# shanpenghui/ExtractORB

Hardware: AMD Instinct MI355X
Metric: frames/sec (ORB extract, 640x480x8-level x1000 feat) (higher is better)
Workload: dtype u8; 1 GPU; mono640: 640x480 mono stream, 8 levels, 1000 features, synthetic noise frames; variant=noise, nfeatures=1000, nlevels=8, handles_per_gpu=1, parallelism=frames sharded 512/GPU

## Files before the change

### extractorb_amd/csrc/k_describe_body.hpp

```cpp
#pragma once
#include <hip/hip_runtime.h>
#include <stdint.h>

#include "orbx_device.hpp"
#include "k_blur_body.hpp"

namespace orbx {
constexpr int kUmaxStatic[16] = {15, 15, 15, 15, 14, 14, 14, 13, 13, 12, 11, 10, 9, 8, 6, 3};
static __constant__ int c_umax[16] = {15, 15, 15, 15, 14, 14, 14, 13, 13, 12, 11, 10, 9, 8, 6, 3};
static __constant__ __attribute__((aligned(16))) float c_patternF[1024] = {
#include "orbx_brief_pattern.inc"
};

__device__ __forceinline__ float fastAtan2Deg(float y, float x) {
    const float sc = (float)(180.0 / 3.1415926535897932384626433832795);
    const float p1 = 0.9997878412794807f * sc, p3 = -0.3258083974640975f * sc, p5 = 0.1555786518463281f * sc,
                p7 = -0.04432655554792128f * sc;
    const float eps = (float)2.2204460492503131e-16;
    const float ax = fabsf(x), ay = fabsf(y);
    float a, c, c2;
    if (ax >= ay) {
        c = __fdiv_rn(ay, __fadd_rn(ax, eps));
        c2 = __fmul_rn(c, c);
        a = __fmul_rn(__fadd_rn(__fmul_rn(__fadd_rn(__fmul_rn(__fadd_rn(__fmul_rn(p7, c2), p5), c2), p3), c2), p1), c);
    } else {
        c = __fdiv_rn(ax, __fadd_rn(ay, eps));
        c2 = __fmul_rn(c, c);
        a = __fsub_rn(90.f, __fmul_rn(__fadd_rn(__fmul_rn(__fadd_rn(__fmul_rn(__fadd_rn(__fmul_rn(p7, c2), p5), c2), p3), c2), p1), c));
    }
    if (x < 0) a = __fsub_rn(180.f, a);
    if (y < 0) a = __fsub_rn(360.f, a);
    return a;
}

__device__ __forceinline__ void sincosGlibc(float y, float* s_out, float* c_out) {
    const double hpi_inv = 0x1.45F306DC9C883p+23, hpi = 0x1.921FB54442D18p0;
    const double C0 = 0x1p0, C1 = -0x1.ffffffd0c621cp-2, C2 = 0x1.55553e1068f19p-5, C3 = -0x1.6c087e89a359dp-10,
                 C4 = 0x1.99343027bf8c3p-16;
    const double S1 = -0x1.555545995a603p-3, S2 = 0x1.1107605230bc4p-7, S3 = -0x1.994eb3774cf24p-13;
    double x = (double)y;
    const unsigned top12 = (__float_as_uint(y) >> 20) & 0x7ff;
    int n = 0;
    if (top12 < 0x3f4) {
        if (top12 < 0x398) { *s_out = y; *c_out = 1.0f; return; }
    } else {
        const double r = __dmul_rn(x, hpi_inv);
        n = ((int)r + 0x800000) >> 24;
        x = __dsub_rn(x, __dmul_rn((double)n, hpi));
    }
    const double x2 = __dmul_rn(x, x);
    auto polySin = [&](double xx) {
        const double x3 = __dmul_rn(xx, x2), s1 = __dadd_rn(S2, __dmul_rn(x2, S3)), x7 = __dmul_rn(x3, x2),
                     s = __dadd_rn(xx, __dmul_rn(x3, S1));
        return __dadd_rn(s, __dmul_rn(x7, s1));
    };
    auto polyCos = [&](double sg) {
        const double x4 = __dmul_rn(x2, x2), c2 = __dadd_rn(sg * C3, __dmul_rn(x2, sg * C4)),
                     c1 = __dadd_rn(sg * C0, __dmul_rn(x2, sg * C1)), x6 = __dmul_rn(x4, x2),
                     c = __dadd_rn(c1, __dmul_rn(x4, sg * C2));
        return __dadd_rn(c, __dmul_rn(x6, c2));
    };
    const bool odd = (n & 1) != 0;
    const int ns = odd ? n + 1 : n, nc = odd ? n : n + 1;
    const double sgnS = ((ns & 3) == 1 || (ns & 3) == 2) ? -1.0 : 1.0;
    const float ps = (float)polySin(x * sgnS), pc = (float)polyCos((nc & 2) ? -1.0 : 1.0);
    *s_out = odd ? pc : ps;
    *c_out = odd ? ps : pc;
}

constexpr int kDescWaves = 4;
constexpr int kBriefReach = 18;
constexpr int kRawRows = 2 * kHalfPatch + 1;
constexpr int kRawStride = 40;
constexpr int kBlurRows = 2 * kBriefReach + 1;
constexpr int kBlurStride = 40;
constexpr int kPatchLds = kRawRows * kRawStride + kBlurRows * kBlurStride;
constexpr int kPbRows = 2 * (kBriefReach + 3) + 1;
constexpr int kPbStride = 44;
constexpr int kPbRawBytes = (kPbRows * kPbStride + 15) & ~15;
constexpr int kPbLds = kPbRawBytes + kBlurRows * kBlurStride;
static __constant__ unsigned c_pbRun[32] = {
    0x0b0700, 0x0c1200, 0x080301, 0x0b0b01, 0x0c1601, 0x0c0102, 0x0c0d02, 0x0b1902, 0x050003, 0x0c0503, 0x091103, 0x0b1a03, 0x050004, 0x0c0504, 0x081104,
    0x0c1904, 0x060005, 0x0c0605, 0x091205, 0x0a1b05, 0x050006, 0x0c0506, 0x0c1106, 0x081d06, 0x0b0207, 0x0b0d07, 0x0b1807, 0x0c0508, 0x0c1108, 0x031d08, 0x010c09, 0x0c0d09};

#if defined(ORBX_DESC_STAMPS) && defined(ORBX_DESCRIBE_TU)
__device__ unsigned long long g_descStamps[6 * 1024];
extern "C" int orbx_debug_desc_stamps(unsigned long long* out) { return (int)hipMemcpyFromSymbol(out, HIP_SYMBOL(g_descStamps), sizeof(g_descStamps)); }
#define DSTAMP(i) do { const int dsW = (int)blockIdx.y * 4 + (int)(threadIdx.x >> 6); \
        if ((threadIdx.x & 63) == 0 && blockIdx.x == 0 && blockIdx.z == 0 && dsW < 1024) g_descStamps[6 * dsW + (i)] = __builtin_amdgcn_s_memrealtime(); } while (0)
#else
#define DSTAMP(i) do {} while (0)
#endif
template <bool PB>
struct DescLds {
    static constexpr int kPatches = 2 * kDescWaves * (PB ? kPbLds : kPatchLds), kWtabWords = 2 * 16 * (PB ? 12 : 8);
    static constexpr int kWtabOff = (kPatches + 15) & ~15, kBytes = kWtabOff + 4 * kWtabWords;
};

template <bool PB>
__device__ __forceinline__ void describeBlock(const LevelGeom* __restrict__ lv, int nlevels,
                                              const uint8_t* __restrict__ pyr, const uint8_t* __restrict__ blur,
                                              const uint2* __restrict__ sel, int selPerFrame,
                                              const int* __restrict__ levelCount, const int* __restrict__ levelLap,
                                              Keypoint* __restrict__ outK, uint8_t* __restrict__ outD, int capacity,
                                              int* __restrict__ nOut, int* __restrict__ monoOut,
                                              Keypoint* __restrict__ outLevelK, int* __restrict__ outLevelCounts, int fewWaves,
                                              uint8_t* smem, unsigned (*wtab)[16][PB ? 12 : 8], int chunk, int f, int levelLo, int levelHi) {
    const int tid = threadIdx.x, wave = tid >> 6, lane = tid & 63, half = lane >> 5, hl = lane & 31;
    DSTAMP(0);
    if constexpr (PB) {
        for (int e = tid; e < 2 * 16 * 12; e += 256) {
            const int which = e / 192, a = (e / 12) & 15, j = e % 12;
            unsigned w = 0;
#pragma unroll
            for (int b = 0; b < 4; b++) {
                const int u = 4 * j + b - (kBriefReach + 4), au = u < 0 ? -u : u;
                if (au <= kHalfPatch && au <= c_umax[a]) w |= (unsigned)(which ? 1 : u + 16) << (8 * b);
            }
            wtab[which][a][j] = w;
        }
    } else {
        const int which = tid >> 7, a = (tid >> 3) & 15, j = tid & 7;
        unsigned w = 0;
#pragma unroll
        for (int b = 0; b < 4; b++) {
            const int u = 4 * j + b - kHalfPatch, au = u < 0 ? -u : u;
            if (au <= c_umax[a]) w |= (unsigned)(which ? 1 : u + 16) << (8 * b);
        }
        wtab[which][a][j] = w;
    }
    __syncthreads();
    const int slot0 = __builtin_amdgcn_readfirstlane((chunk * kDescWaves + wave) * 2);
    const int slot = slot0 + half;
    int total = 0, totalLap = 0, level = 0, seqBase = 0, lapBase = 0, levelN, selOff;
    if (fewWaves) {
        int myOff = 0x7fffffff, myCnt = 0, myLap = 0;
        if (lane < nlevels) { myOff = lv[lane].selOff; myCnt = levelCount[f * nlevels + lane]; myLap = levelLap[f * nlevels + lane]; }
        int incC = myCnt, incL = myLap;
        static_assert(kMaxLevels == 16, "the scan below covers one DPP row of 16 lanes");
        incC += __builtin_amdgcn_update_dpp(0, incC, 0x111, 0xF, 0xF, true); incL += __builtin_amdgcn_update_dpp(0, incL, 0x111, 0xF, 0xF, true);
        incC += __builtin_amdgcn_update_dpp(0, incC, 0x112, 0xF, 0xF, true); incL += __builtin_amdgcn_update_dpp(0, incL, 0x112, 0xF, 0xF, true);
        incC += __builtin_amdgcn_update_dpp(0, incC, 0x114, 0xF, 0xF, true); incL += __builtin_amdgcn_update_dpp(0, incL, 0x114, 0xF, 0xF, true);
        incC += __builtin_amdgcn_update_dpp(0, incC, 0x118, 0xF, 0xF, true); incL += __builtin_amdgcn_update_dpp(0, incL, 0x118, 0xF, 0xF, true);
        total = __builtin_amdgcn_readlane(incC, kMaxLevels - 1); totalLap = __builtin_amdgcn_readlane(incL, kMaxLevels - 1);
        level = __popcll(__ballot(slot0 >= myOff)) - 1;
        seqBase = __builtin_amdgcn_readlane(incC - myCnt, level); lapBase = __builtin_amdgcn_readlane(incL - myLap, level);
        levelN = __builtin_amdgcn_readlane(myCnt, level); selOff = __builtin_amdgcn_readlane(myOff, level);
        if (slot0 == 0 && outLevelCounts && lane < nlevels) outLevelCounts[f * nlevels + lane] = myCnt;
    } else {
        for (int l = 0; l < nlevels; l++) {
            const int c = levelCount[f * nlevels + l], lp = levelLap[f * nlevels + l];
            if (slot0 >= lv[l].selOff) { level = l; seqBase = total; lapBase = totalLap; }
            total += c;
            totalLap += lp;
        }
        selOff = lv[level].selOff;
        levelN = levelCount[f * nlevels + level];
        if (slot0 == 0 && outLevelCounts && lane < nlevels) outLevelCounts[f * nlevels + lane] = levelCount[f * nlevels + lane];
    }
    if (slot0 == 0 && lane == 0) { nOut[f] = total; monoOut[f] = total - totalLap; }
    if (level < levelLo || level >= levelHi) return;
    const int i = slot - selOff;
    const bool active = slot < selPerFrame && i < levelN;
    if (__ballot(active) == 0) return;
    DSTAMP(1);
    const int gw = lv[level].w, gh = lv[level].h, pyrStride = lv[level].pyrStride, blurStride = lv[level].blurStride;
    const uint8_t* pyrL = pyr + lv[level].pyrOff + (long long)f * lv[level].pyrFrameBytes;
    const uint8_t* blurL = blur + lv[level].blurOff + (long long)f * lv[level].blurFrameBytes;
    const uint2 e = active ? sel[(long long)f * selPerFrame + slot] : make_uint2(0u, 0u);
    int kx = e.x & 0xffff, ky = e.x >> 16;
    const float response = (float)(e.y >> 24);
    kx = min(max(kx, kEdge), gw - kEdge - 1);
    ky = min(max(ky, kEdge), gh - kEdge - 1);

    DSTAMP(2);
    int m10 = 0, m01 = 0;
    uint8_t* blurT;
    int blurMis;
    unsigned pbRun = 0;
    if constexpr (PB) pbRun = c_pbRun[hl];
    if constexpr (PB) {
        uint8_t* rawT = smem + (wave * 2 + half) * kPbLds;
        blurT = rawT + kPbRawBytes;
        blurMis = 0;
        constexpr int kSteps = (kPbRows + 3) / 4;
        const int l8 = hl & 7, rsub = hl >> 3;
        const int col0 = kPadL + kx - (kBriefReach + 4), mis = col0 & 3;
        const int rOff = __mul24(kEdge + ky - (kBriefReach + 3) + rsub, pyrStride) + (col0 - mis) + 8 * l8;
        uint2 wr[kSteps];
#pragma unroll
        for (int s = 0; s < kSteps; s++) {
            wr[s] = uint2{0u, 0u};
            if (l8 < 6 && rsub + 4 * s < kPbRows) __builtin_memcpy(&wr[s], pyrL + ((unsigned)rOff + (unsigned)(4 * s * pyrStride)), 8);
        }
        uint8_t* rdst = rawT + rsub * kPbStride + 8 * l8;
#pragma unroll
        for (int s = 0; s < kSteps; s++) {
            const unsigned nxt = (unsigned)__builtin_amdgcn_update_dpp(0, (int)wr[s].x, 0x101, 0xF, 0xF, false);
            const unsigned v0 = __builtin_amdgcn_alignbyte(wr[s].y, wr[s].x, (unsigned)mis), v1 = __builtin_amdgcn_alignbyte(nxt, wr[s].y, (unsigned)mis);
            if (l8 < 6 && rsub + 4 * s < kPbRows) {
                *(unsigned*)(rdst + 4 * s * kPbStride) = v0;
                if (l8 < 5) *(unsigned*)(rdst + 4 * s * kPbStride + 4) = v1;
            }
        }
        asm volatile("" ::: "memory");
        __builtin_amdgcn_fence(__ATOMIC_ACQ_REL, "wavefront");
        __builtin_amdgcn_wave_barrier();
        asm volatile("" ::: "memory");
        DSTAMP(3);
        if (hl < kRawRows) {
            const int v = hl - kHalfPatch, a = v < 0 ? -v : v;
            const unsigned* row = (const unsigned*)(rawT + (hl + 6) * kPbStride);
            unsigned s1 = 0, s0 = 0;
#pragma unroll
            for (int j = 1; j <= 9; j++) {
                const unsigned px = row[j];
                s1 = __builtin_amdgcn_udot4(px, wtab[0][a][j], s1, false);
                s0 = __builtin_amdgcn_udot4(px, wtab[1][a][j], s0, false);
            }
            m10 = (int)s1 - 16 * (int)s0;
            m01 = v * (int)s0;
        }
        {
            const int g4 = (int)(pbRun & 0xff), o0 = (int)((pbRun >> 8) & 0xff), nOut = (int)(pbRun >> 16);
            const uint8_t* src = rawT + o0 * kPbStride + 4 * g4;
            uint8_t* dst = blurT + o0 * kBlurStride + 4 * g4;
            blurRun(nOut,
                    [&](int i, unsigned& d0, unsigned& d1, unsigned& d2) {
                        const unsigned* row = (const unsigned*)(src + min(i, nOut + 5) * kPbStride);
                        d0 = row[0]; d1 = row[1]; d2 = row[2];
                    },
                    [&](int rr, unsigned word) { *(unsigned*)(dst + rr * kBlurStride) = word; });
        }
        asm volatile("" ::: "memory");
        __builtin_amdgcn_fence(__ATOMIC_ACQ_REL, "wavefront");
        __builtin_amdgcn_wave_barrier();
        asm volatile("" ::: "memory");
    } else {
    uint8_t* rawT = smem + (wave * 2 + half) * kPatchLds;
    blurT = rawT + kRawRows * kRawStride;
    const int rawCol0 = kPadL + kx - kHalfPatch, rawMis = rawCol0 & 3;
    const int blurCol0 = kx - kBriefReach;
    blurMis = blurCol0 & 3;
    {
        constexpr int kPairs = 5, kRowsPerStep = 6;
        static_assert(kRawStride == 8 * kPairs && kBlurStride == 8 * kPairs, "tile rows are five 8-byte pairs");
        constexpr int kRawSteps = (kRawRows + kRowsPerStep - 1) / kRowsPerStep, kBlurSteps = (kBlurRows + kRowsPerStep - 1) / kRowsPerStep;
        const int rr = (hl * 52) >> 8, rc = hl - rr * kPairs;
        const bool stLane = hl < kRowsPerStep * kPairs;
        const int rOff = __mul24(kEdge + ky - kHalfPatch + rr, pyrStride) + (rawCol0 - rawMis) + 8 * rc;
        const int bOff = __mul24(ky - kBriefReach + rr, blurStride) + (blurCol0 - blurMis) + 8 * rc;
        uint2 wr[kRawSteps], wb[kBlurSteps];
#pragma unroll
        for (int s = 0; s < kRawSteps; s++) {
            wr[s] = uint2{0u, 0u};
            if (stLane && rr + kRowsPerStep * s < kRawRows) __builtin_memcpy(&wr[s], pyrL + ((unsigned)rOff + (unsigned)(kRowsPerStep * s * pyrStride)), 8);
        }
#pragma unroll
        for (int s = 0; s < kBlurSteps; s++) {
            wb[s] = uint2{0u, 0u};
            if (stLane && rr + kRowsPerStep * s < kBlurRows) __builtin_memcpy(&wb[s], blurL + ((unsigned)bOff + (unsigned)(kRowsPerStep * s * blurStride)), 8);
        }
        uint8_t* rdst = rawT + rr * kRawStride + 8 * rc;
        uint8_t* bdst = blurT + rr * kBlurStride + 8 * rc;
#pragma unroll
        for (int s = 0; s < kRawSteps; s++)
            if (stLane && rr + kRowsPerStep * s < kRawRows) *(uint2*)(rdst + kRowsPerStep * s * kRawStride) = wr[s];
#pragma unroll
        for (int s = 0; s < kBlurSteps; s++)
            if (stLane && rr + kRowsPerStep * s < kBlurRows) *(uint2*)(bdst + kRowsPerStep * s * kBlurStride) = wb[s];
    }
    asm volatile("" ::: "memory");
    __builtin_amdgcn_fence(__ATOMIC_ACQ_REL, "wavefront");
    __builtin_amdgcn_wave_barrier();
    asm volatile("" ::: "memory");

    DSTAMP(3);
    if (hl < kRawRows) {
        const int v = hl - kHalfPatch, a = v < 0 ? -v : v;
        const unsigned* row = (const unsigned*)(rawT + hl * kRawStride);
        unsigned d[9];
#pragma unroll
        for (int j = 0; j < 9; j++) d[j] = row[j];
        unsigned s1 = 0, s0 = 0;
#pragma unroll
        for (int j = 0; j < 8; j++) {
            const unsigned px = __builtin_amdgcn_alignbyte(d[j + 1], d[j], (unsigned)rawMis);
            s1 = __builtin_amdgcn_udot4(px, wtab[0][a][j], s1, false);
            s0 = __builtin_amdgcn_udot4(px, wtab[1][a][j], s0, false);
        }
        m10 = (int)s1 - 16 * (int)s0;
        m01 = v * (int)s0;
    }
    }
    auto rowSum = [](int v) {
        v += __builtin_amdgcn_update_dpp(0, v, 0xB1, 0xF, 0xF, false);
        v += __builtin_amdgcn_update_dpp(0, v, 0x4E, 0xF, 0xF, false);
        v += __builtin_amdgcn_update_dpp(0, v, 0x141, 0xF, 0xF, false);
        v += __builtin_amdgcn_update_dpp(0, v, 0x140, 0xF, 0xF, false);
        return v;
    };
    m10 = rowSum(m10); m01 = rowSum(m01);
    m10 += __shfl_xor(m10, 16);
    m01 += __shfl_xor(m01, 16);
    const float angle = fastAtan2Deg((float)m01, (float)m10);

    const float factorPI = (float)(3.1415926535897932384626433832795 / 180.0);
    float a, b;
    sincosGlibc(__fmul_rn(angle, factorPI), &b, &a);
    const uint8_t* bc = blurT + kBriefReach * kBlurStride + blurMis + kBriefReach;
    unsigned myWord = 0;
#pragma unroll
    for (int j = 0; j < 8; j++) {
        const int p = hl + 32 * j;
        const float4 pt = ((const float4*)c_patternF)[p];
        const float x0 = pt.x, y0 = pt.y, x1 = pt.z, y1 = pt.w;
        const int r0 = (int)rintf(__fadd_rn(__fmul_rn(x0, b), __fmul_rn(y0, a)));
        const int q0 = (int)rintf(__fsub_rn(__fmul_rn(x0, a), __fmul_rn(y0, b)));
        const int r1 = (int)rintf(__fadd_rn(__fmul_rn(x1, b), __fmul_rn(y1, a)));
        const int q1 = (int)rintf(__fsub_rn(__fmul_rn(x1, a), __fmul_rn(y1, b)));
        const int t0 = bc[__mul24(r0, kBlurStride) + q0], t1 = bc[__mul24(r1, kBlurStride) + q1];
        const unsigned long long m = __ballot(t0 < t1);
        const unsigned mine = half ? (unsigned)(m >> 32) : (unsigned)m;
        myWord = hl == j ? mine : myWord;
    }
    DSTAMP(4);
    if (!active) return;

    const int lapRank = (int)(e.y & 0x7fffff), isLap = (int)((e.y >> 23) & 1);
    const int lapBefore = lapBase + lapRank;
    const int monoBefore = (seqBase - lapBase) + (i - lapRank);
    const int at = isLap ? total - 1 - lapBefore : monoBefore;
    float ox = (float)kx, oy = (float)ky;
    const float scale = lv[level].scale;
    if (level != 0) { ox = __fmul_rn(ox, scale); oy = __fmul_rn(oy, scale); }
    const float patchSize = (float)lv[level].patchSize;
    if (at < capacity) {
        if (hl == 0) {
            Keypoint k;
            k.x = ox; k.y = oy; k.size = patchSize; k.angle = angle; k.response = response;
            k.octave = level; k.class_id = -1;
            outK[(long long)f * capacity + at] = k;
        }
        if (hl < 8) ((unsigned*)(outD + ((long long)f * capacity + at) * 32))[hl] = myWord;
    }
    if (outLevelK && hl == 0 && seqBase + i < capacity) {
        Keypoint k;
        k.x = (float)kx; k.y = (float)ky; k.size = patchSize; k.angle = angle; k.response = response;
        k.octave = level; k.class_id = -1;
        outLevelK[(long long)f * capacity + seqBase + i] = k;
    }
}


}
```

### extractorb_amd/csrc/orbx_api.cpp

```cpp
#include "orbx_internal.hpp"

static_assert(sizeof(orbx_keypoint) == sizeof(Keypoint), "orbx_keypoint layout");
static_assert(sizeof(orbx_proj_query) == sizeof(ProjQuery), "orbx_proj_query layout");

double g_hostT[8];
long g_hostN;
const bool g_hostTiming = getenv("ORBX_HOST_TIMING") && atoi(getenv("ORBX_HOST_TIMING")) != 0;
TestAids g_aids;
const char* const kSlotNames[ORBX_NUM_KERNELS] = {"k_pyr_first", "k_resize", "k_blur", "k_fast",
                                            "k_octree", "k_describe", "memset+copies", "batch_total",
                                            "k_stereo_rows+match+filter", "k_frame_finish+k_search_init+k_search_proj"};
thread_local std::string g_createError;

namespace {
constexpr int kSplitRatioNum = 3, kSplitRatioDen = 2;

void freeAll(orbx_handle* h) {
    void* dev[] = {h->d_input, h->d_pyr, h->d_blur, h->d_candPos, h->d_candSeg, h->d_cellCount, h->d_cellOff, h->d_nodeOf, h->d_candCount, h->d_sink, h->d_sel, h->d_levelCount,
                   h->d_levelLap, h->d_lap, h->d_lv, h->d_cells, h->d_rx, h->d_ry, h->d_xq, h->d_cols, h->d_colLevels, h->d_colCoef, h->d_foot, h->d_tiles, h->d_laneItem, h->d_out,
                   h->d_octArena, h->d_leafHist, h->d_leafBest, h->d_leafCode, h->d_bowWord, h->d_bowNode, h->d_bowWeight, h->d_rowOff, h->d_sadDist,
                   h->d_nMatched, h->d_rowList, h->d_uRight, h->d_depth, h->d_clock};
    for (void* p : dev) if (p) (void)hipFree(p);
    if (h->evFork) (void)hipEventDestroy(h->evFork);
    if (h->evJoin) (void)hipEventDestroy(h->evJoin);
// ... 446 lines not shown
int orbx_abi_version(void) { return ORBX_ABI_VERSION; }

const char* orbx_last_error(const orbx_handle* h) { return h ? h->err.c_str() : g_createError.c_str(); }

int orbx_compute_tables(int nfeatures, float scale_factor, int nlevels, float* sf, float* isf, float* s2, float* is2,
                        int* quota, int* umax16) {
    if (nlevels < 1 || nlevels > kMaxLevels || nfeatures < 1 || !(scale_factor > 1.0f)) return ORBX_ERR_BAD_ARGUMENT;
    ScaleTables t = makeScaleTables(nfeatures, scale_factor, nlevels);
    for (int i = 0; i < nlevels; i++) {
        if (sf) sf[i] = t.scale[i];
        if (isf) isf[i] = t.invScale[i];
        if (s2) s2[i] = t.sigma2[i];
        if (is2) is2[i] = t.invSigma2[i];
        if (quota) quota[i] = t.quota[i];
    }
    if (umax16) for (int i = 0; i < 16; i++) umax16[i] = t.umax[i];
    return ORBX_OK;
}

int orbx_compute_level_sizes(float scale_factor, int nlevels, int rows, int cols, int* widths, int* heights) {
    if (nlevels < 1 || nlevels > kMaxLevels || !(scale_factor > 1.0f)) return ORBX_ERR_BAD_ARGUMENT;
    ScaleTables t = makeScaleTables(1000, scale_factor, nlevels);
    for (int l = 0; l < nlevels; l++) {
        widths[l] = roundHalfEven((float)cols * t.invScale[l]);
        heights[l] = roundHalfEven((float)rows * t.invScale[l]);
    }
    return ORBX_OK;
}

int orbx_compute_cell_grid(float scale_factor, int nlevels, int rows, int cols, int level, int* n_cols, int* n_rows,
                           int* w_cell, int* h_cell, int* n_cells, int* n_ini, int* cand_cap) {
    if (nlevels < 1 || nlevels > kMaxLevels || level < 0 || level >= nlevels || !(scale_factor > 1.0f))
        return ORBX_ERR_BAD_ARGUMENT;
    ScaleTables t = makeScaleTables(1000, scale_factor, nlevels);
    FrameGeom g;
    std::string why = makeFrameGeom(t, rows, cols, g);
    if (!why.empty()) return why.find("small") != std::string::npos ? ORBX_ERR_IMAGE_TOO_SMALL : ORBX_ERR_UNSUPPORTED;
    const LevelGeom& L = g.lv[level];
    if (n_cols) *n_cols = L.nCols;
    if (n_rows) *n_rows = L.nRows;
    if (w_cell) *w_cell = L.wCell;
    if (h_cell) *h_cell = L.hCell;
    if (n_cells) *n_cells = L.cellCount;
    if (n_ini) *n_ini = L.nIni;
    if (cand_cap) *cand_cap = L.candCap;
    return ORBX_OK;
}

int orbx_create(orbx_handle** out, int nfeatures, float scale_factor, int nlevels, int ini_th, int min_th,
                int max_width, int max_height, int max_batch, int device) {
    if (!out) return ORBX_ERR_BAD_ARGUMENT;
    *out = nullptr;
    if (nfeatures < 1 || nlevels < 1 || nlevels > kMaxLevels || !(scale_factor > 1.0f) || ini_th < 1 || min_th < 1 ||
        ini_th > 254 || min_th > 254 || max_width < 1 || max_height < 1 || max_batch < 1) {
        g_createError = "orbx_create: bad argument (need nfeatures>=1, 1<=nlevels<=16, scale>1, 1<=thresholds<=254)";
        return ORBX_ERR_BAD_ARGUMENT;
    }
    int ndev = 0;
    if (hipGetDeviceCount(&ndev) != hipSuccess || ndev < 1) {
        g_createError = "orbx_create: no HIP device (this library has no CPU path)";
        return ORBX_ERR_NO_DEVICE;
    }
    orbx_handle* h = new orbx_handle();
    auto bail = [&](int code) {
        g_createError = h->err;
        freeAll(h);
        delete h;
        return code;
    };
#define CREATE_TRY(expr)                                                                 \
    do {                                                                                 \
        hipError_t e_ = (expr);                                                          \
        if (e_ != hipSuccess) {                                                          \
            h->err = std::string(#expr) + ": " + hipGetErrorString(e_);                  \
            return bail(ORBX_ERR_HIP);                                                   \
        }                                                                                \
    } while (0)
    if (device < 0) CREATE_TRY(hipGetDevice(&device));
    if (device >= ndev) { h->err = "orbx_create: device index out of range"; return bail(ORBX_ERR_BAD_ARGUMENT); }
    h->device = device;
    CREATE_TRY(hipSetDevice(device));
    h->nfeatures = nfeatures; h->nlevels = nlevels; h->iniTh = ini_th; h->minTh = min_th; h->scaleFactor = scale_factor;
    h->maxW = max_width; h->maxH = max_height; h->maxB = max_batch;
    h->tabs = makeScaleTables(nfeatures, scale_factor, nlevels);
    auto envInt = [&](const char* name, int dflt) {
        const char* e = getenv(name);
        const int v = e ? atoi(e) : dflt;
        h->policy += std::string(h->policy.empty() ? "" : " ") + (name + 5) + "=" + std::to_string(v) + (e ? "(env)" : "");
        return v;
    };
    std::string why = makeFrameGeom(h->tabs, max_height, max_width, h->maxGeom);
    if (!why.empty()) { h->err = "orbx_create: " + why; return bail(why.find("small") != std::string::npos ? ORBX_ERR_IMAGE_TOO_SMALL : ORBX_ERR_UNSUPPORTED); }
    layoutArenas(h->maxGeom, max_batch);
    const FrameGeom& mg = h->maxGeom;
    auto roomy = [](size_t v) { return v + v / 8 + 4096; };
    h->pyrBytes = roomy((size_t)mg.pyrBytesPerFrame * max_batch);
    h->blurBytes = roomy((size_t)mg.blurBytesPerFrame * max_batch);
    h->candEntries = roomy((size_t)mg.candPerFrame * max_batch);
    h->selEntries = (size_t)(mg.selPerFrame + 8 * nlevels) * max_batch;
    h->cellCap = roomy(mg.cells.size());
    h->rxCap = (size_t)(max_width > max_height ? max_width : max_height) * nlevels + 64;
    h->tileCap = roomy((size_t)(3 * ((max_height + 31) / 32) + (max_height + kBlurBlockRowsSmall - 1) / kBlurBlockRowsSmall + 4) * nlevels);
    h->laneCap = roomy((size_t)((max_width + 3) / 4 + 1) * (3 * ((max_height + 31) / 32) + (max_height + kBlurBlockRowsSmall - 1) / kBlurBlockRowsSmall + 4) * nlevels);
    {
        const OctSizing z = octreeSizing(mg, nlevels, octreeLdsBytes);
        if (z.err) { h->err = std::string("orbx_create: ") + z.err; return bail(ORBX_ERR_UNSUPPORTED); }
        h->octM = z.M; h->octP = z.P; h->octR = z.R; h->octXT = z.XT;
        if (z.arena) {
            h->octArenaSlice = z.arenaSlice;
            if ((double)h->octArenaSlice * max_batch * nlevels > 16e9) {
                h->err = "orbx_create: quad-tree node arena for this nfeatures x max_batch exceeds 16 GB; lower max_batch";
                return bail(ORBX_ERR_UNSUPPORTED);
            }
        }
    }
    h->outCap = mg.selPerFrame + 8 * nlevels;

#define CREATE_ALLOC(ptr, bytes)                                                         \
    do {                                                                                 \
        const size_t n_ = (size_t)(bytes);                                               \
        CREATE_TRY(hipMalloc(&(ptr), n_));                                               \
        if (poison >= 0) CREATE_TRY(hipMemsetAsync((ptr), poison, n_, h->stream));       \
    } while (0)

    const int poison = g_aids.poison >= 0 ? g_aids.poison & 255 : -1;
    CREATE_TRY(hipStreamCreateWithFlags(&h->stream, hipStreamNonBlocking));
    h->ownStream = true;
    CREATE_ALLOC(h->d_input, (size_t)max_width * max_height * max_batch);
    CREATE_ALLOC(h->d_pyr, h->pyrBytes);
    CREATE_ALLOC(h->d_blur, h->blurBytes);
    const size_t candBytes = mg.big ? sizeof(CandFmt<true>::T) : sizeof(CandFmt<false>::T);
    CREATE_ALLOC(h->d_candPos, h->candEntries * candBytes);
    CREATE_ALLOC(h->d_candSeg, h->candEntries * candBytes);
    CREATE_ALLOC(h->d_cellCount, sizeof(unsigned) * h->cellCap * max_batch);
    CREATE_ALLOC(h->d_cellOff, sizeof(int) * h->cellCap * max_batch);
    CREATE_ALLOC(h->d_nodeOf, h->candEntries * sizeof(unsigned short));
    CREATE_ALLOC(h->d_candCount, sizeof(unsigned) * max_batch * nlevels);
    CREATE_ALLOC(h->d_sink, 64);
    CREATE_ALLOC(h->d_sel, h->selEntries * sizeof(uint2));
    if (h->octArenaSlice) CREATE_ALLOC(h->d_octArena, h->octArenaSlice * max_batch * nlevels);
    h->leafFrames = envInt("ORBX_LEAF_FRAMES", 128);
    if (h->leafFrames > max_batch) h->leafFrames = max_batch;
    if (h->octR < 1 || h->octArenaSlice || h->leafFrames < 0) h->leafFrames = 0;
    if (h->leafFrames && (size_t)h->leafFrames * nlevels * h->octR * kOctLeaves >= ((size_t)1 << 30)) h->leafFrames = (int)((((size_t)1 << 30) - 1) / ((size_t)nlevels * h->octR * kOctLeaves));
    if (h->leafFrames) {
        const size_t n = (size_t)h->leafFrames * nlevels * h->octR * kOctLeaves;
        CREATE_ALLOC(h->d_leafHist, n * sizeof(int));
        CREATE_ALLOC(h->d_leafBest, n * sizeof(unsigned));
        CREATE_TRY(hipMemsetAsync(h->d_leafHist, 0, n * sizeof(int), h->stream));
        CREATE_TRY(hipMemsetAsync(h->d_leafBest, 0, n * sizeof(unsigned), h->stream));
        CREATE_ALLOC(h->d_leafCode, (size_t)2 * nlevels * h->octXT);
    }
    CREATE_ALLOC(h->d_levelCount, sizeof(int) * max_batch * nlevels);
    CREATE_ALLOC(h->d_levelLap, sizeof(int) * max_batch * nlevels);
    CREATE_ALLOC(h->d_lap, sizeof(int) * 2 * max_batch);
    CREATE_ALLOC(h->d_lv, sizeof(LevelGeom) * kMaxLevels);
    CREATE_ALLOC(h->d_cells, sizeof(CellDesc) * h->cellCap);
    CREATE_ALLOC(h->d_rx, sizeof(ResizeX) * h->rxCap);
    CREATE_ALLOC(h->d_ry, sizeof(ResizeX) * h->rxCap);
    h->xqCap = ((size_t)(max_width + 2 * kEdge + kPadL) / 4 + 2) * nlevels;
    CREATE_ALLOC(h->d_xq, sizeof(QuadRec) * h->xqCap);
    CREATE_ALLOC(h->d_tiles, sizeof(BlurItem) * h->tileCap);
    CREATE_ALLOC(h->d_laneItem, sizeof(unsigned short) * h->laneCap);
    h->pyrCols = envInt("ORBX_PYR_COLS", -1);
    h->colPx = envInt("ORBX_PYR_COL_PX", 0);
    h->fastWide = envInt("ORBX_FAST_WIDE", -1);
    h->patchBlur = envInt("ORBX_PATCH_BLUR", -1);
    h->blurSplit = envInt("ORBX_BLUR_SPLIT", -1);
    h->sharedUploadBytes = g_aids.sharedUploadBytes;
    h->twoEyesWalk = g_aids.twoEyesWalk == 1;
    h->twoEyesBowStage = g_aids.twoEyesBowStage != 0;
    h->colsShape = g_aids.colsShape == 1 || g_aids.colsShape == 4 || g_aids.colsShape == 6 ? g_aids.colsShape : -1;
    h->colsCap = 0;
    for (int px : kColPx) h->colsCap += (size_t)((max_width + px / 2) / px + 1) * ((max_height + px / 2) / px + 1);
    h->colCoefCap = (h->colsCap + h->colsCap / 8 + 16) * (size_t)kChainCoefMax * 5 / 8;
    h->colsCap = roomy(h->colsCap);
    CREATE_ALLOC(h->d_colCoef, sizeof(ResizeX) * h->colCoefCap);
    CREATE_ALLOC(h->d_cols, sizeof(PyrColumn) * h->colsCap);
    CREATE_ALLOC(h->d_colLevels, sizeof(ColLevels));
    h->footCap = roomy((size_t)((max_width + 38 + 255) / 256 + 1) * ((max_height + 38 + 31) / 32 + 1) * nlevels);
    CREATE_ALLOC(h->d_foot, sizeof(TileFoot) * h->footCap);
    h->outBytes = outLayout(max_batch, h->outCap, nlevels).all;
    CREATE_ALLOC(h->d_out, h->outBytes);
    h->testFailAfterFast = g_aids.failAfterFast != 0;
    g_aids.failAfterFast = 0;
    h->zeroCopy = envInt("ORBX_ZERO_COPY", 1) != 0;
    CREATE_TRY(hipHostMalloc(&h->h_lap, sizeof(int) * 2 * max_batch));
    CREATE_TRY(hipStreamCreateWithFlags(&h->aux, hipStreamNonBlocking));
    CREATE_TRY(hipStreamCreateWithFlags(&h->aux2, hipStreamNonBlocking));
    for (int i = 0; i < 2; i++) { CREATE_TRY(hipEventCreateWithFlags(&h->evPyr[i], hipEventDisableTiming)); CREATE_TRY(hipEventCreateWithFlags(&h->evBlur[i], hipEventDisableTiming)); }
    for (int i = 0; i < 2; i++) CREATE_TRY(hipEventCreateWithFlags(&h->evUp[i], hipEventDisableTiming));
    CREATE_TRY(hipEventCreateWithFlags(&h->evFork, hipEventDisableTiming));
    CREATE_TRY(hipEventCreateWithFlags(&h->evJoin, hipEventDisableTiming));
    h->splitMode = envInt("ORBX_SPLIT", 1);
    h->fuseSmall = envInt("ORBX_FUSE_SMALL", 1) != 0;
    {
        const char* e = getenv("ORBX_SPLIT_MIN_MPX");
        h->splitMinPixels = (long long)((e ? atof(e) : 120.0) * 1e6);
        h->policy += std::string(" SPLIT_MIN_MPX=") + (e ? e : "120") + (e ? "(env)" : "");
    }
    h->resizeBytewise = getenv("ORBX_RESIZE_BYTEWISE") != nullptr;
    h->octRoomyForced = getenv("ORBX_OCT_ROOMY") != nullptr;
    h->policy += std::string(" RESIZE_BYTEWISE=") + (h->resizeBytewise ? "1(env)" : "0") + " OCT_ROOMY=" + (h->octRoomyForced ? "1(env)" : "0");
    h->octThreadsForced = envInt("ORBX_OCT_THREADS", 0);
    if (g_aids.ldsPollute >= 0) h->ldsPollute = g_aids.ldsPollute & 255;
    if (poison >= 0 || h->ldsPollute >= 0 || h->testFailAfterFast || h->colsShape > 0 || h->sharedUploadBytes >= 0)
        h->policy += " test_aids=poison:" + std::to_string(poison) + ",lds_pollute:" + std::to_string(h->ldsPollute) + ",fail_after_fast:" + std::to_string((int)h->testFailAfterFast) +
                     ",pyr_cols_shape:" + std::to_string(h->colsShape) + ",shared_upload_bytes:" + std::to_string(h->sharedUploadBytes);
    {
        int cus = 0;
        if (hipDeviceGetAttribute(&cus, hipDeviceAttributeMultiprocessorCount, h->device) == hipSuccess && cus > 0) h->numCUs = cus;
    }
    CREATE_TRY(hipHostMalloc(&h->h_out, h->outBytes));
    std::memset(h->h_out, 0, h->outBytes);
    h->hInBytes = std::min((size_t)max_width * max_height * max_batch, (size_t)8 << 20);
    CREATE_TRY(hipHostMalloc(&h->h_in, h->hInBytes));
    CREATE_TRY(hipMemsetAsync(h->d_pyr, 0, h->pyrBytes, h->stream));
    CREATE_TRY(hipMemsetAsync(h->d_blur, 0, h->blurBytes, h->stream));
    if (!checkUmax(h->tabs.umax)) { h->err = "orbx_create: the patch-radius table differs from the device's static copy (internal)"; return bail(ORBX_ERR_UNSUPPORTED); }
    {
        unsigned bad = 1;
        CREATE_TRY(runPackedSelfTest(h->stream, (unsigned*)h->d_candCount, &bad));
        if (bad) {
            h->err = "packed min/max self-test failed on this device (FP16 denormals not preserved?): the FAST kernel would not be exact";
            return bail(ORBX_ERR_UNSUPPORTED);
        }
    }
#undef CREATE_TRY
    h->geom = FrameGeom();
    *out = h;
    return ORBX_OK;
}

void orbx_destroy(orbx_handle* h) {
    if (!h) return;
    (void)hipSetDevice(h->device);
    if (h->stream) (void)hipStreamSynchronize(h->stream);
    freeAll(h);
    delete h;
}

int orbx_get_levels(const orbx_handle* h) { return h ? h->nlevels : 0; }
float orbx_get_scale_factor(const orbx_handle* h) { return h ? h->scaleFactor : 0.f; }
int orbx_get_tables(const orbx_handle* h, float* sf, float* isf, float* s2, float* is2, int* quota, int* umax16) {
    if (!h) return ORBX_ERR_BAD_ARGUMENT;
    return orbx_compute_tables(h->nfeatures, h->scaleFactor, h->nlevels, sf, isf, s2, is2, quota, umax16);
}
int orbx_max_keypoints(const orbx_handle* h) { return h ? h->outCap : 0; }

int orbx_set_stream(orbx_handle* h, void* hip_stream) {
    if (!h) return ORBX_ERR_BAD_ARGUMENT;
    HIP_TRY(h, hipSetDevice(h->device));
    if (h->stream) HIP_TRY(h, hipStreamSynchronize(h->stream));
    if (h->ownStream && h->stream) { (void)hipStreamDestroy(h->stream); h->ownStream = false; }
    h->stream = (hipStream_t)hip_stream;
    return ORBX_OK;
}
void* orbx_get_stream(const orbx_handle* h) { return h ? (void*)h->stream : nullptr; }
int orbx_synchronize(orbx_handle* h) {
    if (!h) return ORBX_ERR_BAD_ARGUMENT;
    HIP_TRY(h, hipSetDevice(h->device));
    HIP_TRY(h, hipStreamSynchronize(h->stream));
    return ORBX_OK;
}

int orbx_extract_batch_device(orbx_handle* h, int n_frames, const uint8_t* d_imgs, int rows, int cols,
                              ptrdiff_t stride, ptrdiff_t frame_stride, const int* lap, orbx_keypoint* d_kps,
                              uint8_t* d_desc, int capacity, int* d_n_out, int* d_mono_out, orbx_keypoint* d_level_kps,
                              int* d_level_counts) {
    if (!h) return ORBX_ERR_BAD_ARGUMENT;
    if (!d_imgs || rows <= 0 || cols <= 0) return fail(h, ORBX_ERR_EMPTY_IMAGE, "empty image");
    if (!d_kps || !d_desc || !d_n_out || !d_mono_out || capacity < 1 || stride < cols)
        return fail(h, ORBX_ERR_BAD_ARGUMENT, "null output pointer, capacity < 1 or stride < cols");
    int rc = checkFrameArgs(h, n_frames, rows, cols);
    if (rc != ORBX_OK) return rc;
    return enqueueBatch(h, n_frames, d_imgs, rows, cols, (long long)stride, (long long)frame_stride, lap,
                        (Keypoint*)d_kps, d_desc, capacity, d_n_out, d_mono_out, (Keypoint*)d_level_kps, d_level_counts);
}

int orbx_extract_batch_begin(orbx_handle* h, int n_frames, const uint8_t* imgs, int rows, int cols, ptrdiff_t stride,
                             ptrdiff_t frame_stride, const int* lap, int want_levels) {
    if (!h) return ORBX_ERR_BAD_ARGUMENT;
    if (h->pendingB) return fail(h, ORBX_ERR_BAD_ARGUMENT, "a batch is already in flight on this handle: call orbx_extract_batch_end first");
    if (!imgs || rows <= 0 || cols <= 0) return fail(h, ORBX_ERR_EMPTY_IMAGE, "empty image");
    if (stride < cols) return fail(h, ORBX_ERR_BAD_ARGUMENT, "stride < cols");
    int rc = checkFrameArgs(h, n_frames, rows, cols);
    if (rc != ORBX_OK) return rc;
    HIP_TRY(h, hipSetDevice(h->device));
    hipStream_t st = h->stream;
    const int B = n_frames;
    rc = uploadFrames(h, B, imgs, rows, cols, stride, frame_stride);
    if (rc != ORBX_OK) return rc;
    const int cap = h->outCap;
    const OutLayout lo = outLayout(B, cap, h->nlevels);
    const bool zc = B == 1 && h->zeroCopy;
    h->dev = outView(zc ? h->h_out : h->d_out, lo);
    h->host = outView(h->h_out, lo);
    rc = enqueueBatch(h, B, h->d_input, rows, cols, cols, (long long)rows * cols, lap, h->dev.k, h->dev.d, cap, h->dev.n, h->dev.mono,
                      want_levels ? h->dev.lk : nullptr, want_levels ? h->dev.lc : nullptr);
    if (rc != ORBX_OK) return rc;
    if (!zc) {
        const size_t bytes = want_levels ? lo.all : lo.noLevels;
        if (usesSharedUpload(h, B, rows, cols)) HIP_TRY(h, hipMemcpyAsync(h->h_out, h->d_out, bytes, hipMemcpyDeviceToHost, st));
        else launchCopyOut(st, h->d_out, h->h_out, bytes, h->numCUs);
    }
    h->pendingB = B;
    h->lastHostB = B;
    h->pendingLevels = want_levels != 0;
    return ORBX_OK;
}

int orbx_extract_batch_end(orbx_handle* h, orbx_keypoint* kps, uint8_t* desc, int capacity, int* n_out, int* mono_out,
                           orbx_keypoint* level_kps, int* level_counts) {
    if (!h) return ORBX_ERR_BAD_ARGUMENT;
    if (!h->pendingB) return fail(h, ORBX_ERR_BAD_ARGUMENT, "no batch in flight: call orbx_extract_batch_begin first");
    const int B = h->pendingB, cap = h->outCap;
    h->pendingB = 0;
    if (!kps || !desc || !n_out || !mono_out || capacity < 1) return fail(h, ORBX_ERR_BAD_ARGUMENT, "null output pointer or capacity < 1");
    if ((level_kps || level_counts) && !h->pendingLevels)
        return fail(h, ORBX_ERR_BAD_ARGUMENT, "per-level outputs requested but the batch was begun with want_levels = 0");
    HIP_TRY(h, hipSetDevice(h->device));
    HIP_TRY(h, hipStreamSynchronize(h->stream));
    const orbx_handle::OutView& r = h->host;
    int status = ORBX_OK;
    for (int f = 0; f < B; f++) {
        const int n = r.n[f];
        n_out[f] = n;
        mono_out[f] = r.mono[f];
        if (n > capacity || n > cap) {
            status = fail(h, ORBX_ERR_CAPACITY, "keypoint count exceeds the caller's capacity");
            continue;
        }
        std::memcpy(kps + (size_t)f * capacity, r.k + (size_t)f * cap, (size_t)n * sizeof(Keypoint));
        std::memcpy(desc + (size_t)f * capacity * 32, r.d + (size_t)f * cap * 32, (size_t)n * 32);
        if (level_kps) std::memcpy(level_kps + (size_t)f * capacity, r.lk + (size_t)f * cap, (size_t)n * sizeof(Keypoint));
        if (level_counts) std::memcpy(level_counts + (size_t)f * h->nlevels, r.lc + (size_t)f * h->nlevels, sizeof(int) * h->nlevels);
    }
    return status;
}

int orbx_extract_batch_end_view(orbx_handle* h, const orbx_keypoint** kps, const uint8_t** desc, int* capacity,
                                const int** n_out, const int** mono_out) {
    if (!h) return ORBX_ERR_BAD_ARGUMENT;
    if (!h->pendingB) return fail(h, ORBX_ERR_BAD_ARGUMENT, "no batch in flight: call orbx_extract_batch_begin first");
    h->pendingB = 0;
    if (!kps || !desc || !capacity || !n_out || !mono_out) return fail(h, ORBX_ERR_BAD_ARGUMENT, "null output pointer");
    HIP_TRY(h, hipSetDevice(h->device));
    HIP_TRY(h, hipStreamSynchronize(h->stream));
    *kps = (const orbx_keypoint*)h->host.k; *desc = h->host.d; *capacity = h->outCap;
    *n_out = h->host.n; *mono_out = h->host.mono;
    return ORBX_OK;
}

int orbx_extract_batch(orbx_handle* h, int n_frames, const uint8_t* imgs, int rows, int cols, ptrdiff_t stride,
                       ptrdiff_t frame_stride, const int* lap, orbx_keypoint* kps, uint8_t* desc, int capacity,
                       int* n_out, int* mono_out, orbx_keypoint* level_kps, int* level_counts) {
    if (!h) return ORBX_ERR_BAD_ARGUMENT;
    if (!imgs || rows <= 0 || cols <= 0) return fail(h, ORBX_ERR_EMPTY_IMAGE, "empty image");
    if (!kps || !desc || !n_out || !mono_out || capacity < 1 || stride < cols)
        return fail(h, ORBX_ERR_BAD_ARGUMENT, "null output pointer, capacity < 1 or stride < cols");
    int rc = orbx_extract_batch_begin(h, n_frames, imgs, rows, cols, stride, frame_stride, lap, level_kps || level_counts);
    if (rc != ORBX_OK) return rc;
    return orbx_extract_batch_end(h, kps, desc, capacity, n_out, mono_out, level_kps, level_counts);
}

void* orbx_host_alloc(size_t bytes) {
    void* p = nullptr;
    return hipHostMalloc(&p, bytes) == hipSuccess ? p : nullptr;
}
void orbx_host_free(void* p) { if (p) (void)hipHostFree(p); }

int orbx_extract(orbx_handle* h, const uint8_t* img, int rows, int cols, ptrdiff_t stride, int lap0, int lap1,
                 orbx_keypoint* kps, uint8_t* desc, int capacity, int* n_out, int* mono_out, orbx_keypoint* level_kps,
                 int* level_counts) {
    const int lap[2] = {lap0, lap1};
    return orbx_extract_batch(h, 1, img, rows, cols, stride, (ptrdiff_t)rows * stride, lap, kps, desc, capacity, n_out,
                              mono_out, level_kps, level_counts);
}

int orbx_extract_view(orbx_handle* h, const uint8_t* img, int rows, int cols, ptrdiff_t stride, int lap0, int lap1, int want_levels,
                      const orbx_keypoint** kps, const uint8_t** desc, int* n_out, int* mono_out, const orbx_keypoint** level_kps,
                      const int** level_counts) {
    if (!h) return ORBX_ERR_BAD_ARGUMENT;
    if (!img || rows <= 0 || cols <= 0) return fail(h, ORBX_ERR_EMPTY_IMAGE, "empty image");
    if (!kps || !desc || !n_out || !mono_out || stride < cols || (want_levels && (!level_kps || !level_counts)))
        return fail(h, ORBX_ERR_BAD_ARGUMENT, "null output pointer or stride < cols");
    const int lap[2] = {lap0, lap1};
    const double t0 = g_hostTiming ? nowSec() : 0;
    int rc = orbx_extract_batch_begin(h, 1, img, rows, cols, stride, (ptrdiff_t)rows * stride, lap, want_levels);
    if (rc != ORBX_OK) return rc;
    h->pendingB = 0;
    const double t1 = g_hostTiming ? nowSec() : 0;
    HIP_TRY(h, hipStreamSynchronize(h->stream));
    if (g_hostTiming) { const double t2 = nowSec(); g_hostT[0] += t1 - t0; g_hostT[1] += t2 - t1; g_hostN++; }
    const int n = h->host.n[0];
    if (n < 0 || n > h->outCap) return fail(h, ORBX_ERR_CAPACITY, "keypoint count exceeds the handle's capacity (internal bound violated)");
    *kps = (const orbx_keypoint*)h->host.k; *desc = h->host.d; *n_out = n; *mono_out = h->host.mono[0];
    if (want_levels) { *level_kps = (const orbx_keypoint*)h->host.lk; *level_counts = h->host.lc; }
    return ORBX_OK;
}

int orbx_compute_pyramid(orbx_handle* h, const uint8_t* img, int rows, int cols, ptrdiff_t stride) {
    if (!h) return ORBX_ERR_BAD_ARGUMENT;
    if (h->pendingB) return fail(h, ORBX_ERR_BAD_ARGUMENT, "a batch is already in flight on this handle: call orbx_extract_batch_end first");
    if (!img || rows <= 0 || cols <= 0) return fail(h, ORBX_ERR_EMPTY_IMAGE, "empty image");
    if (stride < cols) return fail(h, ORBX_ERR_BAD_ARGUMENT, "stride < cols");
    int rc = checkFrameArgs(h, 1, rows, cols);
    if (rc != ORBX_OK) return rc;
    HIP_TRY(h, hipSetDevice(h->device));
    rc = uploadFrames(h, 1, img, rows, cols, stride, (ptrdiff_t)rows * stride);
    if (rc != ORBX_OK) return rc;
    rc = enqueueBatch(h, 1, h->d_input, rows, cols, cols, (long long)rows * cols, nullptr, nullptr, nullptr, h->outCap, nullptr, nullptr, nullptr,
                      nullptr, kStageFront);
    if (rc != ORBX_OK) return rc;
    HIP_TRY(h, hipStreamSynchronize(h->stream));
    return ORBX_OK;
}

int orbx_compute_keypoints_octree(orbx_handle* h, orbx_keypoint* level_kps, int capacity, int* level_counts) {
    if (!h) return ORBX_ERR_BAD_ARGUMENT;
    if (!level_kps || !level_counts || capacity < 1) return fail(h, ORBX_ERR_BAD_ARGUMENT, "null output pointer or capacity < 1");
    if (h->pendingB) return fail(h, ORBX_ERR_BAD_ARGUMENT, "a batch is already in flight on this handle: call orbx_extract_batch_end first");
    if (h->geom.nlevels == 0 || h->lastB < 1)
        return fail(h, ORBX_ERR_BAD_ARGUMENT, "orbx_compute_keypoints_octree: the handle holds no pyramid (call orbx_compute_pyramid or an extract call first)");
    HIP_TRY(h, hipSetDevice(h->device));
    const int cap = h->outCap;
    const OutLayout lo = outLayout(1, cap, h->nlevels);
    h->dev = outView(h->zeroCopy ? h->h_out : h->d_out, lo);
    h->host = outView(h->h_out, lo);
    int rc = enqueueBatch(h, 1, h->d_input, h->geom.rows, h->geom.cols, h->geom.cols, (long long)h->geom.rows * h->geom.cols, nullptr, h->dev.k,
                          h->dev.d, cap, h->dev.n, h->dev.mono, h->dev.lk, h->dev.lc, kStageBack);
    if (rc != ORBX_OK) return rc;
    if (!h->zeroCopy) HIP_TRY(h, hipMemcpyAsync(h->h_out, h->d_out, lo.all, hipMemcpyDeviceToHost, h->stream));
    HIP_TRY(h, hipStreamSynchronize(h->stream));
    h->lastHostB = 1;
    const int n = h->host.n[0];
    if (n < 0 || n > cap) return fail(h, ORBX_ERR_CAPACITY, "keypoint count exceeds the handle's capacity (internal bound violated)");
    if (n > capacity) return fail(h, ORBX_ERR_CAPACITY, "keypoint count exceeds the caller's capacity");
    std::memcpy(level_kps, h->host.lk, (size_t)n * sizeof(Keypoint));
    std::memcpy(level_counts, h->host.lc, sizeof(int) * h->nlevels);
    return ORBX_OK;
}

int orbx_fetch_pyramid(orbx_handle* h, int frame, const uint8_t** base, size_t* level_offset, int* level_stride, int* widths, int* heights) {
    if (!h || !base || !level_offset || !level_stride || !widths || !heights) return ORBX_ERR_BAD_ARGUMENT;
    if (h->geom.nlevels == 0 || frame < 0 || frame >= h->lastB)
        return fail(h, ORBX_ERR_BAD_ARGUMENT, "orbx_fetch_pyramid: no such frame in the last batch");
    HIP_TRY(h, hipSetDevice(h->device));
    const FrameGeom& g = h->geom;
    size_t total = 0;
    for (int l = 0; l < g.nlevels; l++) total += (size_t)g.lv[l].pyrFrameBytes;
    if (total > h->hPyrBytes) {
        HIP_TRY(h, hipStreamSynchronize(h->stream));
        if (h->h_pyr) (void)hipHostFree(h->h_pyr);
        h->h_pyr = nullptr; h->hPyrBytes = 0;
        size_t want = 0;
        for (int l = 0; l < h->maxGeom.nlevels; l++) want += (size_t)h->maxGeom.lv[l].pyrStride * h->maxGeom.lv[l].pyrRows;
        want = std::max(want + want / 8 + 4096, total);
        HIP_TRY(h, hipHostMalloc(&h->h_pyr, want));
        h->hPyrBytes = want;
    }
    bool contiguous = true;
    for (int l = 1; l < g.nlevels; l++) contiguous = contiguous && g.lv[l].pyrOff + (long long)frame * g.lv[l].pyrFrameBytes ==
                                                                     g.lv[l - 1].pyrOff + (long long)(frame + 1) * g.lv[l - 1].pyrFrameBytes;
    size_t at = 0;
    for (int l = 0; l < g.nlevels; l++) {
        const LevelGeom& L = g.lv[l];
        if (!contiguous) HIP_TRY(h, hipMemcpyAsync(h->h_pyr + at, h->d_pyr + L.pyrOff + (long long)frame * L.pyrFrameBytes, (size_t)L.pyrFrameBytes, hipMemcpyDeviceToHost, h->stream));
        level_offset[l] = at + (size_t)kEdge * L.pyrStride + kPadL;
        level_stride[l] = L.pyrStride; widths[l] = L.w; heights[l] = L.h;
        at += (size_t)L.pyrFrameBytes;
    }
    if (contiguous) HIP_TRY(h, hipMemcpyAsync(h->h_pyr, h->d_pyr + g.lv[0].pyrOff + (long long)frame * g.lv[0].pyrFrameBytes, total, hipMemcpyDeviceToHost, h->stream));
    HIP_TRY(h, hipStreamSynchronize(h->stream));
    *base = h->h_pyr;
    return ORBX_OK;
}

int orbx_get_level(orbx_handle* h, int frame, int level, int bordered, uint8_t* dst, ptrdiff_t dst_stride, int* width,
                   int* height) {
    if (!h || !dst) return ORBX_ERR_BAD_ARGUMENT;
    if (h->geom.nlevels == 0 || frame < 0 || frame >= h->lastB || level < 0 || level >= h->nlevels)
        return fail(h, ORBX_ERR_BAD_ARGUMENT, "orbx_get_level: no such frame/level in the last batch");
    HIP_TRY(h, hipSetDevice(h->device));
    const LevelGeom& L = h->geom.lv[level];
    const int w = bordered ? L.w + 2 * kEdge : L.w, hh = bordered ? L.h + 2 * kEdge : L.h;
    if (dst_stride < w) return fail(h, ORBX_ERR_BAD_ARGUMENT, "orbx_get_level: dst_stride too small");
    const uint8_t* src = h->d_pyr + L.pyrOff + (long long)frame * L.pyrFrameBytes +
                         (bordered ? (kPadL - kEdge) : ((long long)kEdge * L.pyrStride + kPadL));
    HIP_TRY(h, hipMemcpy2DAsync(dst, dst_stride, src, L.pyrStride, w, hh, hipMemcpyDeviceToHost, h->stream));
    HIP_TRY(h, hipStreamSynchronize(h->stream));
    if (width) *width = L.w;
    if (height) *height = L.h;
    return ORBX_OK;
}

}
```

Baseline: 307,700 frames/s.

## Rewrite per-patch blur with packed udot2 row pairs and magic-number rounding

Replaces the per-lane blurRun over the patch with a new blurPatchLanes routine. It packs horizontal sums of two rows into 16-bit halves and computes the vertical Gaussian taps with udot2, sharing rows across lanes through DPP. A remapped per-lane run table and a new source-offset table assign the work. The BRIEF sampling step swaps rintf plus integer conversion for float magic-number rounding, folded into a raw LDS address calculation. A hipGetLastError check is also added after the copy-out launch. The aim is fewer ALU ops and LDS reads in the describe kernel, at the cost of tricky packed-offset tables and address arithmetic that could be wrong at edge cases.

Result: faster. 312,800 frames/s (median of 6 runs) (+1.7%).

```diff
diff --git a/extractorb_amd/csrc/k_describe_body.hpp b/extractorb_amd/csrc/k_describe_body.hpp
--- a/extractorb_amd/csrc/k_describe_body.hpp
+++ b/extractorb_amd/csrc/k_describe_body.hpp
@@ -80,8 +80,46 @@
 constexpr int kPbRawBytes = (kPbRows * kPbStride + 15) & ~15;
 constexpr int kPbLds = kPbRawBytes + kBlurRows * kBlurStride;
 static __constant__ unsigned c_pbRun[32] = {
-    0x0b0700, 0x0c1200, 0x080301, 0x0b0b01, 0x0c1601, 0x0c0102, 0x0c0d02, 0x0b1902, 0x050003, 0x0c0503, 0x091103, 0x0b1a03, 0x050004, 0x0c0504, 0x081104,
-    0x0c1904, 0x060005, 0x0c0605, 0x091205, 0x0a1b05, 0x050006, 0x0c0506, 0x0c1106, 0x081d06, 0x0b0207, 0x0b0d07, 0x0b1807, 0x0c0508, 0x0c1108, 0x031d08, 0x010c09, 0x0c0d09};
+    0x0c0102, 0x0c0d02, 0x0b1902, 0x060004, 0x0c0604, 0x0c1204, 0x071e04, 0x0a0c09, 0x031609, 0x0c0207, 0x0c0e07, 0x091a07, 0x080003, 0x0c0803, 0x0c1403,
+    0x052003, 0x0c0700, 0x0b1300, 0x060006, 0x0c0606, 0x0c1206, 0x071e06, 0x0a0301, 0x0c0d01, 0x091901, 0x080005, 0x0c0805, 0x0c1405, 0x052005, 0x0c0508,
+    0x0c1108, 0x031d08};
+static __constant__ unsigned c_pbSrc[32] = {
+    0x0621a034, 0x06322244, 0x0642a454, 0x33184664, 0x0628c118, 0x06394328, 0x0649c538, 0x112ee748, 0x063f63ec, 0x0623a074, 0x06342284, 0x0644a494,
+    0x221ae6a4, 0x062b616c, 0x063be37c, 0x064c658c, 0x0629a134, 0x063a2344, 0x33188554, 0x06290120, 0x06398330, 0x064a0540, 0x11218750, 0x06320240,
+    0x06428450, 0x221b2660, 0x062ba174, 0x063c2384, 0x064ca594, 0x0627e0fc, 0x0638630c, 0x0648e51c};
+
+__device__ __forceinline__ void blurPatchLanes(const uint8_t* srcA, const uint8_t* srcB, int split, uint8_t* dst, int kLo, int kHi) {
+    typedef unsigned short u16x2 __attribute__((ext_vector_type(2)));
+    auto dot2 = [](unsigned pair, unsigned short w0, unsigned short w1, unsigned acc) {
+        return __builtin_amdgcn_udot2(__builtin_bit_cast(u16x2, pair), u16x2{w0, w1}, acc, false);
+    };
+    unsigned W[9][4];
+#pragma unroll
+    for (int k = 0; k < 6; k++) {
+        const unsigned* r0 = (const unsigned*)((2 * k < split ? srcA : srcB) + 2 * k * kPbStride);
+        const unsigned* r1 = r0 + kPbStride / 4;
+        unsigned he[4], ho[4];
+        hsums4(r0[0], r0[1], r0[2], he);
+        hsums4(r1[0], r1[1], r1[2], ho);
+#pragma unroll
+        for (int j = 0; j < 4; j++) W[k][j] = (ho[j] << 16) | he[j];
+    }
+#pragma unroll
+    for (int k = 0; k < 3; k++)
+#pragma unroll
+        for (int j = 0; j < 4; j++) W[6 + k][j] = (unsigned)__builtin_amdgcn_update_dpp(0, (int)W[k][j], 0x101, 0xF, 0xF, true);
+#pragma unroll
+    for (int t = 0; t < 6; t++) {
+        unsigned e[4], o[4];
+#pragma unroll
+        for (int j = 0; j < 4; j++) {
+            e[j] = dot2(W[t + 3][j], 18, 0, dot2(W[t + 2][j], 49, 34, dot2(W[t + 1][j], 49, 55, dot2(W[t][j], 18, 34, 32768u))));
+            o[j] = dot2(W[t + 3][j], 34, 18, dot2(W[t + 2][j], 55, 49, dot2(W[t + 1][j], 34, 49, dot2(W[t][j], 0, 18, 32768u))));
+        }
+        if (2 * t >= kLo && 2 * t < kHi) *(unsigned*)(dst + 2 * t * kBlurStride) = satPack4(e);
+        if (2 * t + 1 >= kLo && 2 * t + 1 < kHi) *(unsigned*)(dst + (2 * t + 1) * kBlurStride) = satPack4(o);
+    }
+}
 
 #if defined(ORBX_DESC_STAMPS) && defined(ORBX_DESCRIBE_TU)
 __device__ unsigned long long g_descStamps[6 * 1024];
@@ -177,8 +215,8 @@
     int m10 = 0, m01 = 0;
     uint8_t* blurT;
     int blurMis;
-    unsigned pbRun = 0;
-    if constexpr (PB) pbRun = c_pbRun[hl];
+    unsigned pbRun = 0, pbSrc = 0;
+    if constexpr (PB) { pbRun = c_pbRun[hl]; pbSrc = c_pbSrc[hl]; }
     if constexpr (PB) {
         uint8_t* rawT = smem + (wave * 2 + half) * kPbLds;
         blurT = rawT + kPbRawBytes;
@@ -223,15 +261,11 @@
         }
         {
             const int g4 = (int)(pbRun & 0xff), o0 = (int)((pbRun >> 8) & 0xff), nOut = (int)(pbRun >> 16);
-            const uint8_t* src = rawT + o0 * kPbStride + 4 * g4;
-            uint8_t* dst = blurT + o0 * kBlurStride + 4 * g4;
-            blurRun(nOut,
-                    [&](int i, unsigned& d0, unsigned& d1, unsigned& d2) {
-                        const unsigned* row = (const unsigned*)(src + min(i, nOut + 5) * kPbStride);
-                        d0 = row[0]; d1 = row[1]; d2 = row[2];
-                    },
-                    [&](int rr, unsigned word) { *(unsigned*)(dst + rr * kBlurStride) = word; });
-        }
+            const int k0 = (int)(pbSrc >> 27), split = (int)((pbSrc >> 23) & 15);
+            blurPatchLanes(rawT + (pbSrc & 0x7ff), rawT + ((int)((pbSrc >> 11) & 0xfff) - 1024), split,
+                           blurT + (o0 - k0) * kBlurStride + 4 * g4, k0, k0 + nOut);
+        }
+        DSTAMP(5);
         asm volatile("" ::: "memory");
         __builtin_amdgcn_fence(__ATOMIC_ACQ_REL, "wavefront");
         __builtin_amdgcn_wave_barrier();
@@ -308,18 +342,21 @@
     const float factorPI = (float)(3.1415926535897932384626433832795 / 180.0);
     float a, b;
     sincosGlibc(__fmul_rn(angle, factorPI), &b, &a);
-    const uint8_t* bc = blurT + kBriefReach * kBlurStride + blurMis + kBriefReach;
+    constexpr float kRintMagic = 12582912.f;
+    constexpr unsigned kRintOff = kBlurStride * 0x400000u + 0x4B400000u;
+    typedef __attribute__((address_space(3))) const uint8_t* LdsBytes;
+    const unsigned bc = (unsigned)(uintptr_t)(LdsBytes)(blurT + kBriefReach * kBlurStride + blurMis + kBriefReach) - kRintOff;
     unsigned myWord = 0;
 #pragma unroll
     for (int j = 0; j < 8; j++) {
         const int p = hl + 32 * j;
         const float4 pt = ((const float4*)c_patternF)[p];
         const float x0 = pt.x, y0 = pt.y, x1 = pt.z, y1 = pt.w;
-        const int r0 = (int)rintf(__fadd_rn(__fmul_rn(x0, b), __fmul_rn(y0, a)));
-        const int q0 = (int)rintf(__fsub_rn(__fmul_rn(x0, a), __fmul_rn(y0, b)));
-        const int r1 = (int)rintf(__fadd_rn(__fmul_rn(x1, b), __fmul_rn(y1, a)));
-        const int q1 = (int)rintf(__fsub_rn(__fmul_rn(x1, a), __fmul_rn(y1, b)));
-        const int t0 = bc[__mul24(r0, kBlurStride) + q0], t1 = bc[__mul24(r1, kBlurStride) + q1];
+        const unsigned r0 = __float_as_uint(__fadd_rn(__fadd_rn(__fmul_rn(x0, b), __fmul_rn(y0, a)), kRintMagic));
+        const unsigned q0 = __float_as_uint(__fadd_rn(__fsub_rn(__fmul_rn(x0, a), __fmul_rn(y0, b)), kRintMagic));
+        const unsigned r1 = __float_as_uint(__fadd_rn(__fadd_rn(__fmul_rn(x1, b), __fmul_rn(y1, a)), kRintMagic));
+        const unsigned q1 = __float_as_uint(__fadd_rn(__fsub_rn(__fmul_rn(x1, a), __fmul_rn(y1, b)), kRintMagic));
+        const int t0 = *(LdsBytes)(uintptr_t)(bc + __umul24(r0, kBlurStride) + q0), t1 = *(LdsBytes)(uintptr_t)(bc + __umul24(r1, kBlurStride) + q1);
         const unsigned long long m = __ballot(t0 < t1);
         const unsigned mine = half ? (unsigned)(m >> 32) : (unsigned)m;
         myWord = hl == j ? mine : myWord;
diff --git a/extractorb_amd/csrc/orbx_api.cpp b/extractorb_amd/csrc/orbx_api.cpp
--- a/extractorb_amd/csrc/orbx_api.cpp
+++ b/extractorb_amd/csrc/orbx_api.cpp
@@ -772,7 +772,10 @@
     if (!zc) {
         const size_t bytes = want_levels ? lo.all : lo.noLevels;
         if (usesSharedUpload(h, B, rows, cols)) HIP_TRY(h, hipMemcpyAsync(h->h_out, h->d_out, bytes, hipMemcpyDeviceToHost, st));
-        else launchCopyOut(st, h->d_out, h->h_out, bytes, h->numCUs);
+        else {
+            launchCopyOut(st, h->d_out, h->h_out, bytes, h->numCUs);
+            HIP_TRY(h, hipGetLastError());
+        }
     }
     h->pendingB = B;
     h->lastHostB = B;
```
